# showlab/VideoSwap

Hardware: AMD Instinct MI355X
Metric: denoised frames/sec, 16-frame 512x512 clip @ 50 DDIM steps (end to end: inversion + CFG sampling) (higher is better)
Workload: dtype f16; 1 GPU; BASELINE.json configs[1]: 16-frame 512x512 clip, SD-1.5 UNet3D + AnimateDiff motion modules, 50-step DDIM inversion (B=1) + 50-step CFG-7.5 DDIM sampling (B=2), 1 clip per GPU per step; launch=eager, parallelism=clip-parallel x1

## Files before the change

include/vsx.h:

```cpp
#ifndef VSX_H_
#define VSX_H_

#include <stddef.h>
#include <stdint.h>

#ifdef __cplusplus
extern "C" {
#endif

#define VSX_ABI_VERSION 14

#define VSX_OK 0
#define VSX_E_BADSHAPE (-1)
#define VSX_E_UNSUPPORTED (-2)
#define VSX_E_LAUNCH (-3)
#define VSX_E_WORKSPACE (-4)

typedef void* vsx_stream_t;

int vsx_abi_version(void);
const char* vsx_last_error(void);
const char* vsx_source_digest(void);
int vsx_set_option(const char* name, int64_t value);

// ... 28 lines not shown
    double alpha;
    void* workspace;
    int64_t workspace_bytes;
    int64_t pad_lo, pad_hi;
    const void* rowscale;
    const void* colvec;
    void* rowstats;
    int64_t rowstats_parts;
} vsx_gemm_desc;

int vsx_gemm_f16(const vsx_gemm_desc* d, vsx_stream_t stream);
int64_t vsx_gemm_rowstats_parts(const vsx_gemm_desc* d);
int64_t vsx_gemm_workspace(const vsx_gemm_desc* d);

int64_t vsx_groupnorm_chunks(int64_t rows, int64_t nimg);
int vsx_groupnorm_stats(const void* x1, const void* x2, int64_t nimg, int64_t rows, int64_t C1,
                        int64_t C2, int64_t groups, float* partial, vsx_stream_t stream);
int vsx_groupnorm_apply(const void* x1, const void* x2, int64_t nimg, int64_t rows, int64_t C1,
                        int64_t C2, int64_t groups, const float* partial, int64_t nchunks,
                        int64_t count_rows, const void* gamma, const void* beta, float eps,
                        int64_t silu, float* stats, void* y, vsx_stream_t stream);

int vsx_row_stats(const void* x, int64_t M, int64_t C, float eps, float* stats, vsx_stream_t stream);
int vsx_row_stats_combine(const float* parts, int64_t M, int64_t nparts, int64_t C, float eps, float* stats,
                          vsx_stream_t stream);

int vsx_layernorm(const void* x, int64_t M, int64_t C, const void* gamma, const void* beta,
                  float eps, const void* pe, int64_t rows_per_frame, int64_t frames,
                  int64_t frame_offset, void* y, vsx_stream_t stream);

int vsx_attention_f16(const void* Q, const void* K, const void* VT, void* O, int64_t nb,
                      int64_t heads, int64_t nq, int64_t nk, int64_t d, int64_t ldq, int64_t ldk,
                      int64_t ldvt, int64_t ldo, int64_t q_bs, int64_t k_bs, int64_t vt_bs,
                      int64_t o_bs, int64_t kv_div, float scale, vsx_stream_t stream);

int vsx_attention_lse_f16(const void* Q, const void* K, const void* VT, void* O, float* lse, int64_t lse_ld, int64_t nb,
                          int64_t heads, int64_t nq, int64_t nk, int64_t d, int64_t ldq, int64_t ldk, int64_t ldvt,
                          int64_t ldo, int64_t q_bs, int64_t k_bs, int64_t vt_bs, int64_t o_bs, int64_t kv_div,
                          float scale, vsx_stream_t stream);
int64_t vsx_attention_bwd_supported(int64_t d);
int vsx_attention_bwd_f16(const void* Q, const void* K, const void* V, const void* O, const void* dO, const void* QT,
                          const void* KT, const void* dOT, const float* lse, float* delta, void* dQ, void* dK, void* dV,
                          int64_t nb, int64_t heads, int64_t nq, int64_t nk, int64_t d, int64_t ldtq, int64_t ldtk,
                          int64_t lds, int64_t kv_div, float scale, vsx_stream_t stream);

int vsx_softmax_rows(void* S, int64_t nrows, int64_t ncols, int64_t ld, vsx_stream_t stream);
int vsx_softmax_rows_causal(void* S, int64_t nrows, int64_t ncols, int64_t ld, int64_t rows_per_seq,
                            vsx_stream_t stream);

int vsx_temporal_attention_f16(const void* Q, const void* K, const void* V, void* O, int64_t B,
                               int64_t fq, int64_t fk, int64_t hw, int64_t heads, int64_t d,
                               int64_t ldq, int64_t ldkv, int64_t ldo, float scale,
                               vsx_stream_t stream);

int vsx_silu(const void* x, void* y, int64_t n, vsx_stream_t stream);
int vsx_quick_gelu(const void* x, void* y, int64_t n, vsx_stream_t stream);
int vsx_axpy(const void* a, const void* b, float s, void* y, int64_t n, vsx_stream_t stream);
int vsx_pack_latents(const void* x, void* y, int64_t B, int64_t Cin, int64_t F, int64_t HW,
                     int64_t Cpad, vsx_stream_t stream);
int vsx_unpack_latents(const void* x, void* y, int64_t B, int64_t Cout, int64_t F, int64_t HW,
                       int64_t Cs, vsx_stream_t stream);
int vsx_cfg_ddim_step(const void* x, const void* eps_u, const void* eps_c, float guidance,
                      float alpha_t, float alpha_next, void* out, int64_t n, vsx_stream_t stream);
int vsx_masked_blend(const void* x, const void* src, const void* mask, void* out, int64_t C,
                     int64_t n_sp, vsx_stream_t stream);

int vsx_adapter_scatter(const float* tracks, const int32_t* selected, const void* feat, void* out,
                        int64_t F, int64_t P, int64_t C, int64_t h, int64_t w, float rate,
                        float out_scale, vsx_stream_t stream);

int vsx_prof_enable(int64_t on, int64_t max_samples);
int vsx_prof_pause(int64_t paused);
int vsx_prof_collect(int64_t* n_launches, double* total_ms, double* total_flop);
int vsx_prof_collect_roofline(double peak_flops, double peak_bytes_per_s, int64_t* n_launches, double* total_ms,
                              double* total_flop, double* total_bytes, double* floor_ms, double* byte_bound_ms);

#define VSX_COMM_OP_SEND 1
#define VSX_COMM_OP_RECV 2
#define VSX_COMM_OP_ALLGATHER 3
#define VSX_COMM_OP_ALLREDUCE 4
#define VSX_COMM_OP_LOCAL_COPY 5
#define VSX_COMM_OP_GROUP_START 6
#define VSX_COMM_OP_GROUP_END 7
int vsx_comm_unique_id(void* id128);
int vsx_comm_init(int64_t rank, int64_t nranks, const void* id128);
int vsx_comm_init_recording(int64_t rank, int64_t nranks);
int64_t vsx_comm_recorded(int64_t* out, int64_t capacity);
int64_t vsx_comm_size(void);
int64_t vsx_comm_rank(void);
int vsx_comm_destroy(void);
int vsx_allgather_kv(const void* kv_local, void* kv_all, int64_t batch, int64_t elems_per_batch,
                     vsx_stream_t stream);
int vsx_allgather_f32(const float* local, float* all, int64_t count, vsx_stream_t stream);
int vsx_allreduce_gnstats(float* partial, int64_t count, vsx_stream_t stream);
int vsx_alltoall_f16(const void* send, void* recv, int64_t nouter, int64_t ninner, int64_t block_elems,
                     const int64_t* send_strides, const int64_t* recv_strides, vsx_stream_t stream);

int vsx_geglu_fwd(const void* y2, void* out, int64_t M, int64_t N, vsx_stream_t stream);
int vsx_geglu_bwd(const void* dout, const void* y2, void* dy2, int64_t M, int64_t N, vsx_stream_t stream);
int vsx_silu_bwd(const void* dy, const void* x, void* dx, int64_t n, vsx_stream_t stream);
int64_t vsx_groupnorm_bwd_workspace(int64_t nimg, int64_t rows, int64_t groups);
int vsx_groupnorm_bwd(const void* dy, const void* x1, const void* x2, int64_t nimg, int64_t rows, int64_t C1,
                      int64_t C2, int64_t groups, const void* gamma, const void* beta, float eps, int64_t silu,
                      void* ws, void* dx1, void* dx2, vsx_stream_t stream);
int vsx_layernorm_bwd(const void* dy, const void* x, const void* gamma, float eps, void* dx, int64_t M, int64_t C,
                      vsx_stream_t stream);
// ... 42 lines not shown
```

videoswap_amd/_lib.py:

```python
import ctypes
import os
from ctypes import POINTER, Structure, c_char_p, c_double, c_float, c_int, c_int32, c_int64, c_void_p

_HERE = os.path.dirname(os.path.abspath(__file__))
VARIANT = os.environ.get('VSX_LIB_VARIANT') or None
LIB_PATH = os.path.join(_HERE, 'lib', 'libvsx.so' if not VARIANT else f'libvsx_{VARIANT}.so')

VSX_ABI_VERSION = 14
VSX_E_UNSUPPORTED = -2


class VsxError(RuntimeError):
    pass


class GemmDesc(Structure):

    def __init__(self, *args, **kwargs):
        super().__init__(*args, **kwargs)
        if 'pad_lo' not in kwargs:
            self.pad_lo = -1
        if 'pad_hi' not in kwargs:
            self.pad_hi = -1

    _fields_ = [
        ('M', c_int64), ('N', c_int64), ('K', c_int64),
        ('batch0', c_int64), ('batch1', c_int64),
        ('A', c_void_p), ('A2', c_void_p),
        ('lda', c_int64), ('a_bs0', c_int64), ('a_bs1', c_int64),
        ('a_mode', c_int64), ('H', c_int64), ('W', c_int64), ('C1', c_int64), ('C2', c_int64),
        ('ks', c_int64), ('stride', c_int64), ('upsample', c_int64),
        ('B', c_void_p), ('ldb', c_int64), ('b_bs0', c_int64), ('b_bs1', c_int64),
        ('C', c_void_p), ('ldc', c_int64), ('c_bs0', c_int64), ('c_bs1', c_int64),
        ('c_mode', c_int64), ('c_rows_per_img', c_int64), ('c_img_stride', c_int64),
        ('bias', c_void_p), ('rowvec', c_void_p), ('rows_per_vec', c_int64),
        ('residual', c_void_p), ('ldr', c_int64), ('r_bs0', c_int64), ('r_bs1', c_int64),
        ('geglu', c_int64), ('alpha', c_double),
        ('workspace', c_void_p), ('workspace_bytes', c_int64),
        ('pad_lo', c_int64), ('pad_hi', c_int64),
        ('rowscale', c_void_p), ('colvec', c_void_p),
        ('rowstats', c_void_p), ('rowstats_parts', c_int64),
    ]


PROTOTYPES = {
    'vsx_abi_version': (c_int, []),
    'vsx_last_error': (c_char_p, []),
    'vsx_source_digest': (c_char_p, []),
    'vsx_set_option': (c_int, [c_char_p, c_int64]),
    'vsx_gemm_f16': (c_int, [POINTER(GemmDesc), c_void_p]),
    'vsx_gemm_workspace': (c_int64, [POINTER(GemmDesc)]),
    'vsx_gemm_rowstats_parts': (c_int64, [POINTER(GemmDesc)]),
    'vsx_groupnorm_chunks': (c_int64, [c_int64, c_int64]),
    'vsx_groupnorm_stats': (c_int, [c_void_p, c_void_p, c_int64, c_int64, c_int64, c_int64, c_int64, c_void_p,
                                    c_void_p]),
    'vsx_groupnorm_apply': (c_int, [c_void_p, c_void_p, c_int64, c_int64, c_int64, c_int64, c_int64, c_void_p,
                                    c_int64, c_int64, c_void_p, c_void_p, c_float, c_int64, c_void_p, c_void_p, c_void_p]),
    'vsx_row_stats': (c_int, [c_void_p, c_int64, c_int64, c_float, c_void_p, c_void_p]),
    'vsx_row_stats_combine': (c_int, [c_void_p, c_int64, c_int64, c_int64, c_float, c_void_p, c_void_p]),
    'vsx_layernorm': (c_int, [c_void_p, c_int64, c_int64, c_void_p, c_void_p, c_float, c_void_p, c_int64, c_int64,
                              c_int64, c_void_p, c_void_p]),
    'vsx_attention_f16': (c_int, [c_void_p, c_void_p, c_void_p, c_void_p] + [c_int64] * 14 + [c_float, c_void_p]),
    'vsx_attention_lse_f16': (c_int, [c_void_p, c_void_p, c_void_p, c_void_p, c_void_p] + [c_int64] * 15 + [c_float, c_void_p]),
    'vsx_attention_bwd_supported': (c_int64, [c_int64]),
    'vsx_attention_bwd_f16': (c_int, [c_void_p] * 13 + [c_int64] * 9 + [c_float, c_void_p]),
    'vsx_softmax_rows': (c_int, [c_void_p, c_int64, c_int64, c_int64, c_void_p]),
    'vsx_softmax_rows_causal': (c_int, [c_void_p, c_int64, c_int64, c_int64, c_int64, c_void_p]),
    'vsx_temporal_attention_f16': (c_int, [c_void_p, c_void_p, c_void_p, c_void_p] + [c_int64] * 9
                                   + [c_float, c_void_p]),
    'vsx_silu': (c_int, [c_void_p, c_void_p, c_int64, c_void_p]),
    'vsx_quick_gelu': (c_int, [c_void_p, c_void_p, c_int64, c_void_p]),
    'vsx_axpy': (c_int, [c_void_p, c_void_p, c_float, c_void_p, c_int64, c_void_p]),
    'vsx_pack_latents': (c_int, [c_void_p, c_void_p, c_int64, c_int64, c_int64, c_int64, c_int64, c_void_p]),
    'vsx_unpack_latents': (c_int, [c_void_p, c_void_p, c_int64, c_int64, c_int64, c_int64, c_int64, c_void_p]),
    'vsx_cfg_ddim_step': (c_int, [c_void_p, c_void_p, c_void_p, c_float, c_float, c_float, c_void_p, c_int64,
                                  c_void_p]),
    'vsx_masked_blend': (c_int, [c_void_p, c_void_p, c_void_p, c_void_p, c_int64, c_int64, c_void_p]),
    'vsx_adapter_scatter': (c_int, [c_void_p, c_void_p, c_void_p, c_void_p, c_int64, c_int64, c_int64, c_int64,
                                    c_int64, c_float, c_float, c_void_p]),
    'vsx_prof_enable': (c_int, [c_int64, c_int64]),
    'vsx_comm_unique_id': (c_int, [c_void_p]),
    'vsx_comm_init': (c_int, [c_int64, c_int64, c_void_p]),
    'vsx_comm_init_recording': (c_int, [c_int64, c_int64]),
    'vsx_comm_recorded': (c_int64, [POINTER(c_int64), c_int64]),
    'vsx_comm_size': (c_int64, []),
    'vsx_comm_rank': (c_int64, []),
    'vsx_comm_destroy': (c_int, []),
    'vsx_allgather_kv': (c_int, [c_void_p, c_void_p, c_int64, c_int64, c_void_p]),
    'vsx_allgather_f32': (c_int, [c_void_p, c_void_p, c_int64, c_void_p]),
    'vsx_allreduce_gnstats': (c_int, [c_void_p, c_int64, c_void_p]),
    'vsx_prof_pause': (c_int, [c_int64]),
    'vsx_prof_collect': (c_int, [POINTER(c_int64), POINTER(c_double), POINTER(c_double)]),
    'vsx_prof_collect_roofline': (c_int, [c_double, c_double, POINTER(c_int64), POINTER(c_double), POINTER(c_double),
                                          POINTER(c_double), POINTER(c_double), POINTER(c_double)]),
    'vsx_geglu_fwd': (c_int, [c_void_p, c_void_p, c_int64, c_int64, c_void_p]),
    'vsx_geglu_bwd': (c_int, [c_void_p, c_void_p, c_void_p, c_int64, c_int64, c_void_p]),
    'vsx_silu_bwd': (c_int, [c_void_p, c_void_p, c_void_p, c_int64, c_void_p]),
    'vsx_groupnorm_bwd_workspace': (c_int64, [c_int64, c_int64, c_int64]),
    'vsx_groupnorm_bwd': (c_int, [c_void_p, c_void_p, c_void_p, c_int64, c_int64, c_int64, c_int64, c_int64, c_void_p,
                                  c_void_p, c_float, c_int64, c_void_p, c_void_p, c_void_p, c_void_p]),
    'vsx_layernorm_bwd': (c_int, [c_void_p, c_void_p, c_void_p, c_float, c_void_p, c_int64, c_int64, c_void_p]),
    'vsx_softmax_bwd': (c_int, [c_void_p, c_void_p, c_int64, c_int64, c_int64, c_float, c_void_p]),
    'vsx_sum_pool2x2': (c_int, [c_void_p, c_void_p, c_int64, c_int64, c_int64, c_int64, c_void_p]),
    'vsx_adapter_gather': (c_int, [c_void_p, c_void_p, c_void_p, c_void_p, c_int64, c_int64, c_int64, c_int64, c_int64,
                                   c_float, c_float, c_void_p]),
    'vsx_alltoall_f16': (c_int, [c_void_p, c_void_p, c_int64, c_int64, c_int64, POINTER(c_int64), POINTER(c_int64),
                                 c_void_p]),
    'vsx_dift_sample_points': (c_int, [c_void_p] + [c_int64] * 7 + [c_void_p, c_int64, c_void_p, c_int64, c_void_p,
                                                                       c_void_p, c_void_p]),
    'vsx_dift_cosine_map_workspace': (c_int64, [c_int64] * 5),
    'vsx_dift_cosine_map': (c_int, [c_void_p] + [c_int64] * 7 + [c_void_p, c_int64, c_int64, c_void_p, c_int64,
                                                                    c_void_p, c_void_p, c_void_p, c_void_p]),
    'vsx_coord_mlp_f32': (c_int, [c_void_p] + [c_int64] * 10 + [c_void_p, c_int64, c_void_p, c_void_p]),
    'vsx_hash_grid_geometry': (c_int64, [c_int64] * 4 + [c_double] + [c_void_p] * 5),
    'vsx_hash_grid_f32': (c_int, [c_void_p, c_int64, c_int64, c_void_p] + [c_int64] * 5 + [c_double, c_void_p, c_void_p]),
    'vsx_hash_mlp_f32': (c_int, [c_void_p, c_int64, c_int64, c_void_p] + [c_int64] * 5 + [c_double] + [c_int64] * 5
                         + [c_void_p, c_int64, c_void_p, c_void_p]),
    'vsx_atlas_edit_f32': (c_int, [c_void_p, c_void_p, c_void_p, c_int64]
                           + ([c_void_p] + [c_int64] * 3 + [c_float] * 3 + [c_void_p, c_void_p, c_int64, c_int64]) * 2
                           + [c_void_p] * 5),
}

# ... 43 lines not shown
```

videoswap_amd/attention.py:

```python
import torch
from torch import nn

from . import ops
from .layers import Identity, Linear, StepInvariantCache


class Attention(nn.Module):
    def __init__(self, query_dim, cross_attention_dim=None, heads=8, dim_head=64, dropout=0.0, bias=False,
                 upcast_attention=False, upcast_softmax=False, out_bias=True, scale_qk=True,
                 only_cross_attention=False, rescale_output_factor=1.0, residual_connection=False, processor=None,
                 **unsupported):
        super().__init__()
        if upcast_attention or upcast_softmax or dropout != 0.0 or unsupported:
            raise NotImplementedError(f'Attention: unsupported options {unsupported or "upcast/dropout"}')
        inner_dim = dim_head * heads
        cross_attention_dim = cross_attention_dim if cross_attention_dim is not None else query_dim
        self.upcast_attention = False
        self.upcast_softmax = False
        self.rescale_output_factor = rescale_output_factor
        self.residual_connection = residual_connection
        self.scale_qk = scale_qk
        self.scale = dim_head ** -0.5 if scale_qk else 1.0
        self.heads = heads
        self.sliceable_head_dim = heads
# ... 177 lines not shown
        return self.pe[0]


class VanillaAttentionProcessor(nn.Module):
    vsx_native = True

    @property
    def vsx_graph_safe(self):
        return self.kv_gather is None

    def __init__(self, attention_mode=None, cross_frame_attention_mode=None, temporal_position_encoding=False,
                 temporal_position_encoding_max_len=24, attention_op=None, *args, **kwargs):
        super().__init__()
        self.attention_op = attention_op
        self.attention_mode = attention_mode
        self.is_cross_attention = kwargs.get('cross_attention_dim') is not None
        if attention_mode != 'Temporal' or self.is_cross_attention:
            raise NotImplementedError('only Temporal_Self attention blocks exist in the VideoSwap configs')
        self.pos_encoder = PositionalEncoding(kwargs['query_dim'], dropout=0.0,
                                              max_len=temporal_position_encoding_max_len) \
            if temporal_position_encoding else None
        self.kv_gather = None

    @property
    def frame_offset(self):
        g = self.kv_gather
        return g.frame_offset if g is not None and g.kv_active else 0

    def pe_table(self):
        return None if self.pos_encoder is None else self.pos_encoder.table()

    def __call__(self, attn, hidden_states, encoder_hidden_states=None, attention_mask=None, temb=None,
                 video_length=None, residual=None, pe_applied=False):
        bf, hw, c = hidden_states.shape
        frames = video_length
        b = bf // frames
        x = hidden_states
        if self.pos_encoder is not None and not pe_applied:
            pe = self.pe_table()[self.frame_offset:self.frame_offset + frames].to(x.dtype)
            x = (x.view(b, frames, hw, c) + pe[None, :, None, :]).view(bf, hw, c)
        nobias = attn.to_q.bias is None and attn.to_k.bias is None and attn.to_v.bias is None
        fk = frames
        if self.kv_gather is not None and self.kv_gather.kv_active:
            if nobias:
                kv = ops.linear(x, attn.fused_weight(('to_k', 'to_v'))).view(-1, 2 * c)
            else:
                kv = torch.cat([attn.to_k(x).view(-1, c), attn.to_v(x).view(-1, c)], dim=1)
            handle = self.kv_gather.kv_gather_start(kv, b, frames, hw)
            q = attn.to_q(x).view(-1, c)
            kv_all, fk = self.kv_gather.kv_gather_finish(handle)
            k, v = kv_all[:, :c], kv_all[:, c:]
        elif nobias:
            qkv = ops.linear(x, attn.fused_weight(('to_q', 'to_k', 'to_v'))).view(-1, 3 * c)
            q, k, v = qkv[:, :c], qkv[:, c:2 * c], qkv[:, 2 * c:]
        else:
            q, k, v = attn.to_q(x).view(-1, c), attn.to_k(x).view(-1, c), attn.to_v(x).view(-1, c)
        o = ops.temporal_attention(q, k, v, b, frames, fk, hw, attn.heads, attn.scale).view(bf, hw, c)
        return attn.to_out[0](o, residual=residual, row_stats=True)
```

videoswap_amd/build.py:

```python
import hashlib
import os
import re
import shutil
import subprocess
import sys
import tempfile
from concurrent.futures import ThreadPoolExecutor

HERE = os.path.dirname(os.path.abspath(__file__))
ROOT = os.path.dirname(HERE)
CSRC = os.path.join(HERE, 'csrc')
LIBDIR = os.path.join(HERE, 'lib')
OBJDIR = os.path.join(LIBDIR, 'obj')
LIB = os.path.join(LIBDIR, 'libvsx.so')
VARIANTS = {}
VARIANT_EXTRA = {}
SOURCES = ['api.cpp', 'comm.cpp', 'options.cpp', 'prof.cpp', 'gemm.hip', 'gemm_pp.hip', 'norm.hip', 'attention.hip', 'attention_bwd.hip', 'elementwise.hip',
           'train.hip', 'dift.hip', 'atlas.hip', 'atlas_edit.hip']
HIPCC = os.environ.get('HIPCC', '/opt/rocm/bin/hipcc')
FLAGS = ['--offload-arch=gfx950', '-O3', '-std=c++17', '-fPIC', '-x', 'hip',
         '-I', os.path.join(ROOT, 'include'), '-I', CSRC, '-Wall', '-Wno-unused-function', '-Wno-division-by-zero',
         '-mllvm', '-amdgpu-mfma-vgpr-form']


def lib_path(variant=None):
    return LIB if not variant else os.path.join(LIBDIR, f'libvsx_{variant}.so')


def _digest(variant=None):
    h = hashlib.sha256()
    swap = VARIANTS[variant] if variant else {}
    names = [n for n in sorted(os.listdir(CSRC)) if n.endswith(('.hip', '.cpp', '.h'))]
    for name in names + ['../../include/vsx.h']:
        with open(os.path.join(CSRC, swap.get(name, name)), 'rb') as f:
            h.update(name.encode() + b'\0' + f.read())
    h.update(' '.join(f.replace(ROOT, '<root>') for f in FLAGS).encode())
    if variant:
        for name in VARIANT_EXTRA.get(variant, []):
            with open(os.path.join(CSRC, name), 'rb') as f:
                h.update(name.encode() + b'\0' + f.read())
        h.update(b'\0variant ' + variant.encode())
    return h.hexdigest()


def source_digest(variant=None):
    return _digest(variant)


_MARKER = b'@vsx-source-digest:'


def built_digest(variant=None):
    path = lib_path(variant)
    if not os.path.exists(path):
        return None
    with open(path, 'rb') as f:
        blob = f.read()
    i = blob.find(_MARKER)
    if i < 0:
        return None
    j = blob.find(b'\0', i)
    return blob[i + len(_MARKER):j].decode(errors='replace')


def _compile(src, digest, variant=None):
    objdir = OBJDIR if not variant else os.path.join(LIBDIR, f'obj_{variant}')
    os.makedirs(objdir, exist_ok=True)
    obj = os.path.join(objdir, src.replace('/', '_') + '.o')
    extra = [f'-DVSX_SOURCE_DIGEST="{digest}"'] if src == 'api.cpp' else []
    path = os.path.join(CSRC, (VARIANTS[variant] if variant else {}).get(src, src))
    cmd = [HIPCC] + FLAGS + extra + ['-c', path, '-o', obj]
    r = subprocess.run(cmd, capture_output=True, text=True)
    if r.returncode != 0:
        raise RuntimeError(f'hipcc failed for {src}:\n{r.stdout}\n{r.stderr}')
    if r.stderr.strip():
        sys.stderr.write(r.stderr)
    return obj


LLVM_BIN = os.environ.get('VSX_LLVM_BIN', '/opt/rocm/lib/llvm/bin')
NO_SCRATCH = ('gemm_pp_kernel', 'gemm_ws320_kernel', 'flash_attn_kernel', 'gemm_kernelILi256E', 'coord_mlp_kernel')


def parse_kernel_notes(text):
    keys = ('vgpr_count', 'agpr_count', 'sgpr_count', 'vgpr_spill_count', 'sgpr_spill_count',
            'private_segment_fixed_size', 'group_segment_fixed_size')
    out, cur = {}, None
    for line in text.splitlines():
        m = re.match(r'^\s+(-\s+)?\.(\w+):\s*(\S.*)?$', line)
        if not m:
            continue
        if m.group(1) and re.match(r'^  - ', line):
            cur = {}
        if cur is None:
            continue
        key, val = m.group(2), (m.group(3) or '').strip()
        if key == 'name' and re.match(r'^    \.name:', line):
            out[val] = cur
        elif key in keys and re.match(r'^  (- |  )\.', line):
            cur[key] = int(val)
    return out


def kernel_resources(lib=None):
    lib = lib or LIB
    objdump, readelf = os.path.join(LLVM_BIN, 'llvm-objdump'), os.path.join(LLVM_BIN, 'llvm-readelf')
    tmp = tempfile.mkdtemp(prefix='vsx_co_')
    try:
        copy = os.path.join(tmp, 'lib.so')
        shutil.copy(lib, copy)
        r = subprocess.run([objdump, '--offloading', copy], capture_output=True, text=True, cwd=tmp)
        if r.returncode != 0:
            raise RuntimeError(f'llvm-objdump --offloading failed:\n{r.stderr}')
        res = {}
        for name in sorted(os.listdir(tmp)):
            if 'gfx950' not in name:
                continue
            r = subprocess.run([readelf, '--notes', os.path.join(tmp, name)], capture_output=True, text=True)
            if r.returncode != 0:
                raise RuntimeError(f'llvm-readelf --notes failed on {name}:\n{r.stderr}')
            res.update(parse_kernel_notes(r.stdout))
        return res
    finally:
        shutil.rmtree(tmp, ignore_errors=True)


def demangle(names):
    filt = shutil.which('c++filt') or shutil.which('llvm-cxxfilt')
    out = []
    if filt and names:
        r = subprocess.run([filt], input='\n'.join(names), capture_output=True, text=True)
        out = r.stdout.splitlines() if r.returncode == 0 else []
    return dict(zip(names, out if len(out) == len(names) else names))

# ... 126 lines not shown
```

videoswap_amd/csrc/options.cpp:

```cpp
#include "options.h"

#include <stdlib.h>
#include <string.h>

#include "common.h"

namespace vsxg {
namespace {
struct Option { const char* name; const char* env; long value; bool init; };
Option g_options[] = {{"gemm_pp", "VSX_GEMM_PP", 1, false}, {"pp_sched", "VSX_PP_SCHED", 0, false},
                      {"tile_tune", "VSX_TUNE_TILE", 0, false}, {"xcd_walk", "VSX_XCD_WALK", 1, false},
                      {"attn_qb", "VSX_ATTN_QB", 0, false}, {"temporal_out", "VSX_TEMPORAL_OUT", 0, false},
                      {"attn_o16", "VSX_ATTN_O16", 0, false}, {"gn_fuse", "VSX_GN_FUSE", 0, false},
                      {"gemm_ws", "VSX_GEMM_WS", 1, false}, {"ws_waves", "VSX_WS_WAVES", 10, false}};
Option* find_option(const char* name) {
    for (auto& o : g_options)
        if (strcmp(o.name, name) == 0) {
            if (!o.init) {
                const char* e = getenv(o.env);
                if (e) o.value = atol(e);
                o.init = true;
            }
            return &o;
        }
    return nullptr;
}
}
long gemm_option(const char* name) {
    Option* o = find_option(name);
    return o ? o->value : 0;
}
}

extern "C" int vsx_set_option(const char* name, int64_t value) {
    auto* o = name ? vsxg::find_option(name) : nullptr;
    if (!o) return vsx_fail(VSX_E_BADSHAPE, "vsx_set_option: unknown option '%s'", name ? name : "(null)");
    o->value = (long)value;
    return VSX_OK;
}
```

videoswap_amd/ops.py:

```python
import ctypes
import os

import torch

from . import _lib
from ._lib import GemmDesc, check

_F16 = torch.float16


_raw_stream = getattr(torch._C, '_cuda_getCurrentRawStream', None)


def _stream():
    if _raw_stream is not None:
        return ctypes.c_void_p(_raw_stream(torch.cuda.current_device()))
    return ctypes.c_void_p(torch.cuda.current_stream().cuda_stream)


def _p(t):
    return None if t is None else ctypes.c_void_p(t.data_ptr())


def _chk(t, name, dtype=_F16):
# ... 452 lines not shown
    _chk_view(t, name)
    if t.dim() != 3 or t.stride(2) != 1 or t.stride(1) % 8 or t.stride(0) % 8 or (t.data_ptr() % 16):
        raise _lib.VsxError(f'{name}: need unit inner stride, 16-byte aligned base, strides multiple of 8 (got {t.stride()})')
    return t.stride(1), t.stride(0)


def _chk_view(t, name):
    if not t.is_cuda or t.dtype != _F16:
        raise _lib.VsxError(f'{name}: expected an fp16 GPU tensor')


def attention(q, k, vt, heads, scale, kv_div=1, nk=None):
    _chk(vt, 'vt')
    ldq, q_bs = _rows_view(q, 'q')
    ldk, k_bs = _rows_view(k, 'k')
    nb, nq, C = q.shape
    nk = k.shape[1] if nk is None else nk
    dh = C // heads
    out = torch.empty(nb, nq, C, dtype=_F16, device=q.device)
    if FlopCounter.enabled:
        FlopCounter.attention += 4.0 * nb * heads * nq * nk * dh
    check(_lib.load().vsx_attention_f16(_p(q), _p(k), _p(vt), _p(out), nb, heads, nq, nk, dh, ldq, ldk, vt.shape[2], C,
                                        q_bs, k_bs, C * vt.shape[2], nq * C, kv_div, float(scale),
                                        _stream()), 'vsx_attention_f16')
    return out


def temporal_attention(q, k, v, B, fq, fk, hw, heads, scale):
    for t, n in ((q, 'q'), (k, 'k'), (v, 'v')):
        _chk_view(t, n)
        if t.dim() != 2 or t.stride(1) != 1 or t.stride(0) % 8 or t.data_ptr() % 16:
            raise _lib.VsxError(f'{n}: need a [rows, C] tensor with unit inner stride and aligned rows')
    if k.stride(0) != v.stride(0):
        raise _lib.VsxError('temporal_attention: k and v must share their row stride')
    C = q.shape[-1]
    out = torch.empty(q.shape[0], C, dtype=_F16, device=q.device)
    if FlopCounter.enabled:
        FlopCounter.attention += 4.0 * B * hw * fq * fk * C
    fn = _lib.load().vsx_temporal_attention_f16
    if fq <= 32 or fk > 128:
        check(fn(_p(q), _p(k), _p(v), _p(out), B, fq, fk, hw, heads, C // heads, q.stride(0), k.stride(0), C,
                 float(scale), _stream()), 'vsx_temporal_attention_f16')
        return out
    for b in range(B):
        kb, vb = k[b * fk * hw:(b + 1) * fk * hw], v[b * fk * hw:(b + 1) * fk * hw]
        for f0 in range(0, fq, 32):
            n = min(32, fq - f0)
            r0 = (b * fq + f0) * hw
            check(fn(_p(q[r0:r0 + n * hw]), _p(kb), _p(vb), _p(out[r0:r0 + n * hw]), 1, n, fk, hw, heads, C // heads,
                     q.stride(0), k.stride(0), C, float(scale), _stream()), 'vsx_temporal_attention_f16')
    return out


def group_norm(x, gamma, beta, groups, eps, nimg, silu=False, x2=None, partial_hook=None, count_rows=None):
    _chk(x, 'x'); _chk(x2, 'x2'); _chk(gamma, 'gamma'); _chk(beta, 'beta')
    C1 = x.shape[-1]
    C2 = x2.shape[-1] if x2 is not None else 0
    rows = x.numel() // C1 // nimg
    lib = _lib.load()
    nchunks = lib.vsx_groupnorm_chunks(rows, nimg)
    partial = torch.empty(nimg, nchunks, groups, 2, dtype=torch.float32, device=x.device)
    s = _stream()
    check(lib.vsx_groupnorm_stats(_p(x), _p(x2), nimg, rows, C1, C2, groups, _p(partial), s), 'vsx_groupnorm_stats')
    if partial_hook is not None:
        partial = partial_hook(partial)
        nchunks = partial.shape[1]
    y = torch.empty(*x.shape[:-1], C1 + C2, dtype=_F16, device=x.device)
    stats = torch.empty(nimg, groups, 2, dtype=torch.float32, device=x.device)
    check(lib.vsx_groupnorm_apply(_p(x), _p(x2), nimg, rows, C1, C2, groups, _p(partial), nchunks,
                                  rows if count_rows is None else count_rows, _p(gamma), _p(beta), float(eps),
                                  1 if silu else 0, _p(stats), _p(y), s), 'vsx_groupnorm_apply')
    return y


def layer_norm(x, gamma, beta, eps=1e-5, pe=None, rows_per_frame=0, frames=0, frame_offset=0):
    if isinstance(x, DeferredLN):
        raise _lib.VsxError('layer_norm of a deferred LayerNorm: materialize() it first')
    _chk(x, 'x'); _chk(gamma, 'gamma'); _chk(beta, 'beta'); _chk(pe, 'pe')
    C = x.shape[-1]
    if pe is not None:
        if pe.dim() != 2 or pe.shape[1] != C or frames <= 0 or rows_per_frame <= 0 or frame_offset < 0 \
                or pe.shape[0] < frame_offset + frames:
            raise _lib.VsxError(f'layer_norm: positional-encoding table {tuple(pe.shape)} does not cover frames '
                                f'[{frame_offset}, {frame_offset + frames}) x {C} channels')
    y = torch.empty_like(x)
    check(_lib.load().vsx_layernorm(_p(x), x.numel() // C, C, _p(gamma), _p(beta), float(eps), _p(pe), rows_per_frame,
                                    frames, frame_offset, _p(y), _stream()), 'vsx_layernorm')
    return y


def silu(x):
    _chk(x, 'x')
    y = torch.empty_like(x)
    check(_lib.load().vsx_silu(_p(x), _p(y), x.numel(), _stream()), 'vsx_silu')
    return y


def quick_gelu(x):
    _chk(x, 'x')
    y = torch.empty_like(x)
    check(_lib.load().vsx_quick_gelu(_p(x), _p(y), x.numel(), _stream()), 'vsx_quick_gelu')
    return y


def axpy(a, b, s=1.0):
    _chk(a, 'a'); _chk(b, 'b')
# ... 427 lines not shown
```

Measured before the change: 4.274 frames/s.

## Fuse temporal attention with output projection, bias, residual and row stats for C=320

Adds a persistent HIP kernel for the 320-channel, 8-head, 16-frame temporal attention blocks. Each block loads packed q|k|v rows into LDS, runs attention with MFMA, then multiplies by the to_out weight held in registers. The same kernel adds bias and residual and writes per-row statistics for the following layernorm. This removes the separate attention-output round trip through HBM and the extra GEMM and epilogue launches, at the cost of a highly specialized kernel with tight LDS and register budgets that only applies to large M (>=65536) by default.

```diff
diff --git a/include/vsx.h b/include/vsx.h
--- a/include/vsx.h
+++ b/include/vsx.h
@@ -104,6 +104,10 @@
                                int64_t fq, int64_t fk, int64_t hw, int64_t heads, int64_t d,
                                int64_t ldq, int64_t ldkv, int64_t ldo, float scale,
                                vsx_stream_t stream);
+int vsx_temporal_attention_out_f16(const void* Q, const void* K, const void* V, int64_t ldq, int64_t ldkv, const void* W,
+                                   const void* bias, const void* residual, int64_t ldr, void* out, int64_t ldo,
+                                   float* rowstats, int64_t rowstats_parts, int64_t b, int64_t frames, int64_t hw,
+                                   int64_t heads, int64_t d, float scale, vsx_stream_t stream);
 
 int vsx_silu(const void* x, void* y, int64_t n, vsx_stream_t stream);
 int vsx_quick_gelu(const void* x, void* y, int64_t n, vsx_stream_t stream);
diff --git a/videoswap_amd/_lib.py b/videoswap_amd/_lib.py
--- a/videoswap_amd/_lib.py
+++ b/videoswap_amd/_lib.py
@@ -68,6 +68,8 @@
     'vsx_softmax_rows_causal': (c_int, [c_void_p, c_int64, c_int64, c_int64, c_int64, c_void_p]),
     'vsx_temporal_attention_f16': (c_int, [c_void_p, c_void_p, c_void_p, c_void_p] + [c_int64] * 9
                                    + [c_float, c_void_p]),
+    'vsx_temporal_attention_out_f16': (c_int, [c_void_p, c_void_p, c_void_p, c_int64, c_int64, c_void_p, c_void_p, c_void_p,
+                                               c_int64, c_void_p, c_int64, c_void_p] + [c_int64] * 6 + [c_float, c_void_p]),
     'vsx_silu': (c_int, [c_void_p, c_void_p, c_int64, c_void_p]),
     'vsx_quick_gelu': (c_int, [c_void_p, c_void_p, c_int64, c_void_p]),
     'vsx_axpy': (c_int, [c_void_p, c_void_p, c_float, c_void_p, c_int64, c_void_p]),
diff --git a/videoswap_amd/attention.py b/videoswap_amd/attention.py
--- a/videoswap_amd/attention.py
+++ b/videoswap_amd/attention.py
@@ -253,6 +253,14 @@
             k, v = kv_all[:, :c], kv_all[:, c:]
         elif nobias:
             qkv = ops.linear(x, attn.fused_weight(('to_q', 'to_k', 'to_v'))).view(-1, 3 * c)
+            to_out = attn.to_out[0]
+            if (c == 320 and attn.heads == 8 and frames == 16 and residual is not None and ops.ROW_STATS_FROM_PRODUCER and qkv.is_cuda
+                    and type(to_out) is Linear and not (torch.is_grad_enabled() and (
+                        qkv.requires_grad or residual.requires_grad or to_out.weight.requires_grad))):
+                out = ops.temporal_attention_out(qkv, to_out.weight, to_out.bias, residual, b, frames, hw, attn.heads,
+                                                 attn.scale, shape=(bf, hw, c))
+                if out is not None:
+                    return out
             q, k, v = qkv[:, :c], qkv[:, c:2 * c], qkv[:, 2 * c:]
         else:
             q, k, v = attn.to_q(x).view(-1, c), attn.to_k(x).view(-1, c), attn.to_v(x).view(-1, c)
diff --git a/videoswap_amd/build.py b/videoswap_amd/build.py
--- a/videoswap_amd/build.py
+++ b/videoswap_amd/build.py
@@ -15,7 +15,7 @@
 LIB = os.path.join(LIBDIR, 'libvsx.so')
 VARIANTS = {}
 VARIANT_EXTRA = {}
-SOURCES = ['api.cpp', 'comm.cpp', 'options.cpp', 'prof.cpp', 'gemm.hip', 'gemm_pp.hip', 'norm.hip', 'attention.hip', 'attention_bwd.hip', 'elementwise.hip',
+SOURCES = ['api.cpp', 'comm.cpp', 'options.cpp', 'prof.cpp', 'gemm.hip', 'gemm_pp.hip', 'norm.hip', 'attention.hip', 'temporal_out.hip', 'attention_bwd.hip', 'elementwise.hip',
            'train.hip', 'dift.hip', 'atlas.hip', 'atlas_edit.hip']
 HIPCC = os.environ.get('HIPCC', '/opt/rocm/bin/hipcc')
 FLAGS = ['--offload-arch=gfx950', '-O3', '-std=c++17', '-fPIC', '-x', 'hip',
@@ -79,7 +79,7 @@
 
 
 LLVM_BIN = os.environ.get('VSX_LLVM_BIN', '/opt/rocm/lib/llvm/bin')
-NO_SCRATCH = ('gemm_pp_kernel', 'gemm_ws320_kernel', 'flash_attn_kernel', 'gemm_kernelILi256E', 'coord_mlp_kernel')
+NO_SCRATCH = ('gemm_pp_kernel', 'gemm_ws320_kernel', 'flash_attn_kernel', 'gemm_kernelILi256E', 'coord_mlp_kernel', 'temporal_out320_kernel')
 
 
 def parse_kernel_notes(text):
diff --git a/videoswap_amd/csrc/options.cpp b/videoswap_amd/csrc/options.cpp
--- a/videoswap_amd/csrc/options.cpp
+++ b/videoswap_amd/csrc/options.cpp
@@ -12,7 +12,8 @@
                       {"tile_tune", "VSX_TUNE_TILE", 0, false}, {"xcd_walk", "VSX_XCD_WALK", 1, false},
                       {"attn_qb", "VSX_ATTN_QB", 0, false}, {"temporal_out", "VSX_TEMPORAL_OUT", 0, false},
                       {"attn_o16", "VSX_ATTN_O16", 0, false}, {"gn_fuse", "VSX_GN_FUSE", 0, false},
-                      {"gemm_ws", "VSX_GEMM_WS", 1, false}, {"ws_waves", "VSX_WS_WAVES", 10, false}};
+                      {"gemm_ws", "VSX_GEMM_WS", 1, false}, {"ws_waves", "VSX_WS_WAVES", 10, false},
+                      {"temporal_fuse", "VSX_TEMPORAL_FUSE", 1, false}};
 Option* find_option(const char* name) {
     for (auto& o : g_options)
         if (strcmp(o.name, name) == 0) {
diff --git a/videoswap_amd/csrc/temporal_out.hip b/videoswap_amd/csrc/temporal_out.hip
--- /dev/null
+++ b/videoswap_amd/csrc/temporal_out.hip
@@ -0,0 +1,379 @@
+#include "gemm_common.h"
+
+namespace vsxg {
+namespace {
+
+struct TempOutParams {
+    const half_t* QKV;
+    const half_t* W;
+    const half_t* bias;
+    const half_t* residual;
+    half_t* out;
+    float* rowstats;
+    long ldr, ldo;
+    int parts;
+    int hw, bph, nblocks;
+    unsigned qkv_bytes;
+    float sl2;
+};
+
+constexpr int TO_NW = 10;
+constexpr int TO_F = 16, TO_D = 40, TO_C = 320;
+constexpr int TO_ROWB = 3 * TO_C * 2;
+constexpr int TO_FRB = 2 * TO_ROWB;
+constexpr int TO_SLOT = TO_F * TO_FRB;
+constexpr int TO_XP = TO_SLOT / 1024 / TO_NW;
+constexpr int TO_OT = 32 * 640;
+constexpr int TO_VT = 2 * 32 * 40 * 2;
+constexpr int TO_STG = 32 * 36 * 4;
+constexpr int TO_EXTRA = 2 * TO_SLOT;
+constexpr int TO_CST = TO_EXTRA + 2 * TO_STG;
+constexpr int TO_LDS = TO_CST + TO_NW * 128;
+constexpr int TO_WREG = 3 * 32 * 128;
+static_assert(TO_XP * TO_NW * 1024 == TO_SLOT, "the pieces of a block divide evenly among the waves");
+static_assert(TO_OT + 8 * TO_VT <= TO_SLOT && TO_STG <= TO_VT, "o tile and V^T / staging areas fit the slot being computed");
+static_assert(TO_NW * TO_WREG <= 2 * TO_SLOT && TO_LDS <= 160 * 1024, "LDS budget");
+
+__device__ __forceinline__ int to_fresh_lane(const int lane_hint) {
+    int l = lane_hint;
+    asm volatile("v_mbcnt_lo_u32_b32 %0, -1, 0\n\tv_mbcnt_hi_u32_b32 %0, -1, %0" : "=v"(l));
+    return l;
+}
+
+__device__ __forceinline__ int to_chunk(const int f, const int w) { return f * 3840 + ((w ^ f) << 4); }
+
+__device__ __forceinline__ int to_vt_col(const int key, const int chgroup) { return key ^ ((chgroup & 3) << 3); }
+
+__global__ __launch_bounds__(TO_NW * 64) void temporal_out320_kernel(const TempOutParams p) {
+    constexpr int RL = 2;
+    constexpr int OOB_OFF = (int)0x80000000;
+    constexpr int VSTR = 40;
+    extern __shared__ __attribute__((aligned(16))) unsigned char smem[];
+    const int tid = threadIdx.x;
+    const int lane = tid & 63;
+    const int wave = __builtin_amdgcn_readfirstlane(tid >> 6);
+    const int l31 = lane & 31, hi = lane >> 5;
+    const int lrow = lane >> 3, pslot = lane & 7;
+    const int chain = blockIdx.x, nchains = gridDim.x;
+    const int hw = p.hw, bph = p.bph;
+    int nmine = 0;
+    if (chain < p.nblocks) nmine = (p.nblocks - 1 - chain) / nchains + 1;
+    if (nmine == 0) return;
+
+    h8 wf[20];
+    {
+        const __amdgpu_buffer_rsrc_t rsrcW = __builtin_amdgcn_make_buffer_rsrc(const_cast<half_t*>(p.W), 0, TO_C * TO_C * 2, 0x00020000);
+        const int vw_e = lrow * (TO_C * 2) + (pslot ^ (lrow >> 1)) * 16;
+        const int vw_o = lrow * (TO_C * 2) + (pslot ^ (4 | (lrow >> 1))) * 16;
+        unsigned char* wreg = smem + wave * TO_WREG;
+        const int fw = l31 * 128 + ((hi ^ ((l31 >> 1) & 7)) * 16);
+        auto w_round = [&](const int sl0, const int nsl) {
+#pragma unroll
+            for (int sl = 0; sl < 3; ++sl)
+                if (sl < nsl)
+#pragma unroll
+                    for (int pc = 0; pc < 4; ++pc)
+                        __builtin_amdgcn_raw_ptr_buffer_load_lds(rsrcW, (lptr_t)(wreg + sl * 4096 + pc * 1024), 16, (pc & 1) ? vw_o : vw_e,
+                                                                 (32 * wave + 8 * pc) * (TO_C * 2) + (sl0 + sl) * 128, 0, 0);
+            wait_vmcnt<0>();
+            __builtin_amdgcn_sched_barrier(0);
+        };
+        w_round(0, 3);
+#pragma unroll
+        for (int t = 0; t < 12; ++t) wf[t] = *reinterpret_cast<const h8*>(wreg + (t >> 2) * 4096 + (fw ^ ((t & 3) * 32)));
+        asm volatile("s_waitcnt lgkmcnt(0)" ::: "memory");
+        __builtin_amdgcn_sched_barrier(0);
+        w_round(3, 2);
+#pragma unroll
+        for (int t = 12; t < 20; ++t) wf[t] = *reinterpret_cast<const h8*>(wreg + ((t >> 2) - 3) * 4096 + (fw ^ ((t & 3) * 32)));
+        asm volatile("s_waitcnt lgkmcnt(0)" ::: "memory");
+    }
+    const bool has_bias = p.bias != nullptr;
+    float* cst = reinterpret_cast<float*>(smem + TO_CST + wave * 128);
+    if (has_bias && lane < 8) {
+        const h4 cb = *reinterpret_cast<const h4*>(p.bias + 32 * wave + 4 * lane);
+        f4v bf;
+#pragma unroll
+        for (int e = 0; e < 4; ++e) bf[e] = (float)cb[e];
+        *reinterpret_cast<f4v*>(cst + 4 * lane) = bf;
+    }
+    __builtin_amdgcn_sched_barrier(0);
+    __builtin_amdgcn_s_barrier();
+    __builtin_amdgcn_sched_barrier(0);
+
+    const __amdgpu_buffer_rsrc_t rsrcX = __builtin_amdgcn_make_buffer_rsrc(const_cast<half_t*>(p.QKV), 0, (int)p.qkv_bytes, 0x00020000);
+    const unsigned frame_b = (unsigned)hw * (unsigned)TO_ROWB;
+    auto block_coords = [&](const int i, unsigned& row0, bool& two) {
+        const int blk = chain + i * nchains;
+        const int b = blk / bph, jj = blk - b * bph;
+        row0 = (unsigned)(b * TO_F) * (unsigned)hw + 2u * (unsigned)jj;
+        two = 2 * jj + 1 < hw;
+    };
+    auto issue_x = [&](const int i, const int lane) {
+        const bool on = i < nmine;
+        unsigned row0 = 0;
+        bool two = false;
+        block_coords(on ? i : 0, row0, two);
+        const unsigned base = row0 * (unsigned)TO_ROWB;
+        const int slot = (i & 1) * TO_SLOT;
+#pragma unroll
+        for (int k = 0; k < TO_XP; ++k) {
+            const int c = (wave * TO_XP + k) * 64 + lane;
+            const int f = c / 240, w = (c - f * 240) ^ f;
+            const bool take = on && (two || w < 120);
+            __builtin_amdgcn_raw_ptr_buffer_load_lds(rsrcX, (lptr_t)(smem + slot + (wave * TO_XP + k) * 1024), 16,
+                                                     take ? (int)(base + (unsigned)f * frame_b + (unsigned)w * 16u) : OOB_OFF, 0, 0, 0);
+        }
+    };
+    issue_x(0, lane);
+    wait_vmcnt<0>();
+
+    const int asite = min(wave >> 2, 1), head0 = (wave & 3) * 2;
+    unsigned char* priv = smem + (wave < 8 ? TO_OT + wave * TO_VT : TO_EXTRA + (wave - 8) * TO_STG);
+    const int lane_entry = lane;
+
+    int prev_stores = 0;
+    for (int j = 0; j < nmine; ++j) {
+        const int lane = to_fresh_lane(lane_entry);
+        const int l31 = lane & 31, hi = lane >> 5;
+        const int fa = l31 * 128 + ((hi ^ ((l31 >> 1) & 7)) * 16);
+        const int col8 = (lane & 3) * 8, r0 = lane >> 2;
+        const int ncol = 32 * wave + col8;
+        if (j > 0) {
+            if (prev_stores == 4) wait_vmcnt<4>();
+            else wait_vmcnt<2>();
+        }
+        __builtin_amdgcn_sched_barrier(0);
+        __builtin_amdgcn_s_barrier();
+        __builtin_amdgcn_sched_barrier(0);
+        unsigned row0 = 0;
+        bool two = false;
+        block_coords(j, row0, two);
+        h8 pre[RL];
+#pragma unroll
+        for (int ps = 0; ps < RL; ++ps) {
+            const size_t m = (size_t)row0 + (size_t)r0 * (unsigned)hw + (two ? ps : 0);
+            pre[ps] = *reinterpret_cast<const h8*>(p.residual + m * (size_t)p.ldr + ncol);
+        }
+        VSX_VMEM_NOTE(RL);
+        asm volatile("" ::: "memory");
+        __builtin_amdgcn_sched_barrier(0);
+        issue_x(j + 1, lane);
+        unsigned char* slot = smem + (j & 1) * TO_SLOT;
+        float* stg = reinterpret_cast<float*>(wave < 8 ? slot + (priv - smem) : priv);
+
+        const unsigned char* xs = slot;
+        const int wsite = asite * (TO_ROWB / 16);
+        h8 raw[3];
+        h8 ka[3], qb[3];
+        const int krow = (l31 & ~12) | ((l31 & 4) << 1) | ((l31 & 8) >> 1);
+        const int qg = l31 >> 4, qf_ = l31 & 15;
+        {
+#pragma unroll
+            for (int i = 0; i < 3; ++i) {
+                const int u = min(lane + 64 * i, 159);
+                const int key = u / 5, ch = u - key * 5;
+                const int g = key >> 4, f = key & 15;
+                raw[i] = *reinterpret_cast<const h8*>(xs + to_chunk(f, wsite + 80 + (head0 + g) * 5 + ch));
+            }
+            const int kg = krow >> 4, kf_ = krow & 15;
+            const int kw = wsite + 40 + (head0 + kg) * 5 + hi, qw = wsite + (head0 + qg) * 5 + hi;
+#pragma unroll
+            for (int t = 0; t < 3; ++t) {
+                const bool in = t * 16 + hi * 8 < TO_D;
+                const h8 kv = *reinterpret_cast<const h8*>(xs + to_chunk(kf_, kw + 2 * t)), qv = *reinterpret_cast<const h8*>(xs + to_chunk(qf_, qw + 2 * t));
+                ka[t] = in ? kv : h8{};
+                qb[t] = in ? qv : h8{};
+            }
+        }
+        asm volatile("s_waitcnt lgkmcnt(0)" ::: "memory");
+        __builtin_amdgcn_sched_barrier(0);
+        __builtin_amdgcn_s_barrier();
+        __builtin_amdgcn_sched_barrier(0);
+
+        if (wave < 8) {
+            half_t* sVT = reinterpret_cast<half_t*>(stg);
+#pragma unroll
+            for (int i = 0; i < 3; ++i) {
+                const int u = lane + 64 * i;
+                if (u < 160) {
+                    const int key = u / 5, ch = u - key * 5;
+                    const h8 v = raw[i];
+#pragma unroll
+                    for (int e = 0; e < 8; ++e) sVT[(ch * 8 + e) * VSTR + to_vt_col(key, ch)] = v[e];
+                }
+            }
+            const f16v zero = {0.f, 0.f, 0.f, 0.f, 0.f, 0.f, 0.f, 0.f, 0.f, 0.f, 0.f, 0.f, 0.f, 0.f, 0.f, 0.f};
+            f16v sc = zero;
+#pragma unroll
+            for (int t = 0; t < 3; ++t) sc = __builtin_amdgcn_mfma_f32_32x32x16_f16(ka[t], qb[t], t == 0 ? zero : sc, 0, 0, 0);
+            const int lo = qg * TO_F, up = lo + TO_F;
+            const float sl2 = p.sl2;
+            float mx = -INFINITY;
+#pragma unroll
+            for (int r = 0; r < 16; ++r) {
+                const int key = (r & 3) + 4 * ((r >> 2) & 1) + 8 * hi + 16 * (r >> 3);
+                const bool v = key >= lo && key < up;
+                sc[r] = v ? sc[r] * sl2 : -INFINITY;
+                mx = fmaxf(mx, sc[r]);
+            }
+            mx = fmaxf(mx, __shfl_xor(mx, 32, 64));
+            if (mx == -INFINITY) mx = 0.f;
+            float sum = 0.f;
+#pragma unroll
+            for (int r = 0; r < 16; ++r) {
+                sc[r] = __builtin_amdgcn_exp2f(sc[r] - mx);
+                sum += sc[r];
+            }
+            sum += __shfl_xor(sum, 32, 64);
+            const float inv = sum > 0.f ? 1.0f / sum : 0.f;
+            h8 pf[2];
+#pragma unroll
+            for (int s2 = 0; s2 < 2; ++s2)
+#pragma unroll
+                for (int jj = 0; jj < 8; ++jj) pf[s2][jj] = (half_t)sc[8 * s2 + jj];
+            __builtin_amdgcn_sched_barrier(0);
+            const int orow = asite * 16 + qf_;
+            unsigned char* ot = slot + orow * 128;
+            const int osw = (orow >> 1) & 7;
+#pragma unroll
+            for (int t = 0; t < 2; ++t) {
+                f16v o = zero;
+#pragma unroll
+                for (int s2 = 0; s2 < 2; ++s2) {
+                    const h8 vf = *reinterpret_cast<const h8*>(sVT + (t * 32 + l31) * VSTR + to_vt_col(16 * s2 + 8 * hi, (t * 32 + l31) >> 3));
+                    o = __builtin_amdgcn_mfma_f32_32x32x16_f16(vf, pf[s2], o, 0, 0, 0);
+                }
+#pragma unroll
+                for (int g4 = 0; g4 < 4; ++g4) {
+                    const int c = t * 32 + 8 * g4 + 4 * hi;
+                    if (c < TO_D) {
+                        h4 pk;
+#pragma unroll
+                        for (int e = 0; e < 4; ++e) pk[e] = (half_t)(o[4 * g4 + e] * inv);
+                        const int col = (head0 + qg) * TO_D + c;
+                        *reinterpret_cast<h4*>(ot + (col >> 6) * 4096 + ((((col & 63) >> 3) ^ osw) * 16) + (col & 7) * 2) = pk;
+                    }
+                }
+            }
+        }
+        asm volatile("s_waitcnt lgkmcnt(0)" ::: "memory");
+        __builtin_amdgcn_sched_barrier(0);
+        __builtin_amdgcn_s_barrier();
+        __builtin_amdgcn_sched_barrier(0);
+
+        f16v acc;
+        {
+            const f16v zero = {};
+            const h8 xf = *reinterpret_cast<const h8*>(slot + fa);
+            acc = __builtin_amdgcn_mfma_f32_32x32x16_f16(wf[0], xf, zero, 0, 0, 0);
+        }
+#pragma unroll
+        for (int t = 1; t < 20; ++t) {
+            const h8 xf = *reinterpret_cast<const h8*>(slot + (t >> 2) * 4096 + (fa ^ ((t & 3) * 32)));
+            acc = __builtin_amdgcn_mfma_f32_32x32x16_f16(wf[t], xf, acc, 0, 0, 0);
+        }
+#pragma unroll
+        for (int g = 0; g < 4; ++g) {
+            f4v v;
+#pragma unroll
+            for (int e = 0; e < 4; ++e) v[e] = acc[4 * g + e] * 1.0f;
+            *reinterpret_cast<f4v*>(stg + l31 * 36 + 8 * g + 4 * hi) = v;
+        }
+        __builtin_amdgcn_sched_barrier(0);
+        float bv[8];
+        if (has_bias) {
+            const f4v b0 = *reinterpret_cast<const f4v*>(cst + col8), b1 = *reinterpret_cast<const f4v*>(cst + col8 + 4);
+#pragma unroll
+            for (int e = 0; e < 4; ++e) { bv[e] = b0[e]; bv[e + 4] = b1[e]; }
+        }
+#pragma unroll
+        for (int ps = 0; ps < 2; ++ps) {
+            const int row = ps * 16 + r0;
+            const f4v a = *reinterpret_cast<const f4v*>(stg + row * 36 + col8);
+            const f4v b = *reinterpret_cast<const f4v*>(stg + row * 36 + col8 + 4);
+            float ov[8] = {a[0], a[1], a[2], a[3], b[0], b[1], b[2], b[3]};
+            if (has_bias) {
+#pragma unroll
+                for (int e = 0; e < 8; ++e) ov[e] += bv[e];
+            }
+            const h8 add = pre[ps];
+#pragma unroll
+            for (int e = 0; e < 8; ++e) ov[e] += (float)add[e];
+            h8 pk;
+#pragma unroll
+            for (int e = 0; e < 8; ++e) pk[e] = (half_t)ov[e];
+            const h2 one2 = {(half_t)1.f, (half_t)1.f};
+            float s1 = 0.f, s2 = 0.f;
+#pragma unroll
+            for (int e = 0; e < 8; e += 2) {
+                const h2 v = {pk[e], pk[e + 1]};
+                s1 = __builtin_amdgcn_fdot2(v, one2, s1, false);
+                s2 = __builtin_amdgcn_fdot2(v, v, s2, false);
+            }
+#pragma unroll
+            for (int d = 2; d > 0; d >>= 1) {
+                s1 += __shfl_xor(s1, d, 64);
+                s2 += __shfl_xor(s2, d, 64);
+            }
+            if (ps == 0 || two) {
+                const size_t m = (size_t)row0 + (size_t)r0 * (unsigned)hw + ps;
+                *reinterpret_cast<h8*>(p.out + m * (size_t)p.ldo + ncol) = pk;
+                typedef float f2v __attribute__((ext_vector_type(2)));
+                float* sp = p.rowstats + (m * (unsigned)p.parts + (unsigned)wave) * 2;
+                if (col8 == 0) *reinterpret_cast<f2v*>(sp) = f2v{s1, s2};
+            }
+        }
+        prev_stores = two ? 4 : 2;
+        VSX_VMEM_NOTE(prev_stores);
+        __builtin_amdgcn_sched_barrier(0);
+    }
+}
+
+}
+}
+
+extern "C" int vsx_temporal_attention_out_f16(const void* Q, const void* K, const void* V, int64_t ldq, int64_t ldkv, const void* W,
+                                              const void* bias, const void* residual, int64_t ldr, void* out, int64_t ldo,
+                                              float* rowstats, int64_t rowstats_parts, int64_t b, int64_t frames, int64_t hw,
+                                              int64_t heads, int64_t d, float scale, vsx_stream_t stream) {
+    using namespace vsxg;
+    VSX_REQUIRE(Q && K && V && W && out, VSX_E_BADSHAPE, "temporal_attention_out: null tensor");
+    VSX_REQUIRE(b >= 0 && hw >= 0 && frames > 0 && heads > 0 && d > 0, VSX_E_BADSHAPE, "temporal_attention_out: bad sizes");
+    const long fuse = gemm_option("temporal_fuse");
+    const long M = (long)(b * frames * hw);
+    const half_t* q = (const half_t*)Q;
+    const bool shape = heads == 8 && d == TO_D && frames == TO_F && ldq == 3 * TO_C && ldkv == 3 * TO_C &&
+                       (const half_t*)K == q + TO_C && (const half_t*)V == q + 2 * TO_C && residual != nullptr && rowstats != nullptr &&
+                       rowstats_parts == TO_NW && ldr >= TO_C && ldo >= TO_C && ldr % 8 == 0 && ldo % 8 == 0 && vsx_aligned16(Q) &&
+                       vsx_aligned16(W) && vsx_aligned16(bias) && vsx_aligned16(residual) && vsx_aligned16(out) &&
+                       ((uintptr_t)rowstats & 7) == 0 && (unsigned long)M * TO_ROWB < (1ul << 31) &&
+                       (unsigned long)M * (unsigned long)(ldr > ldo ? ldr : ldo) * 2ul < (1ul << 40);
+    if (!shape || fuse == 0 || (fuse == 1 && M < 65536))
+        return vsx_fail(VSX_E_UNSUPPORTED, "temporal_attention_out: not the fused shape (C = 320, 8 heads of 40, 16 frames, q|k|v in one "
+                                           "[M, 960] buffer, residual and 10 statistics parts) or temporal_fuse = %ld", fuse);
+    if (M == 0) return VSX_OK;
+    static bool attr_set = false;
+    if (!attr_set) {
+        hipError_t e = hipFuncSetAttribute(reinterpret_cast<const void*>(&temporal_out320_kernel), hipFuncAttributeMaxDynamicSharedMemorySize, TO_LDS);
+        if (e != hipSuccess) return vsx_fail(VSX_E_LAUNCH, "temporal_attention_out: hipFuncSetAttribute: %s", hipGetErrorString(e));
+        attr_set = true;
+    }
+    static int n_cu = 0;
+    if (n_cu == 0) {
+        int dev = 0;
+        hipDeviceProp_t prop;
+        if (hipGetDevice(&dev) != hipSuccess || hipGetDeviceProperties(&prop, dev) != hipSuccess)
+            return vsx_fail(VSX_E_LAUNCH, "temporal_attention_out: cannot query the device");
+        n_cu = prop.multiProcessorCount > 0 ? prop.multiProcessorCount : 256;
+    }
+    TempOutParams p;
+    p.QKV = q; p.W = (const half_t*)W; p.bias = (const half_t*)bias; p.residual = (const half_t*)residual;
+    p.out = (half_t*)out; p.rowstats = rowstats; p.ldr = ldr; p.ldo = ldo; p.parts = (int)rowstats_parts;
+    p.hw = (int)hw; p.bph = (int)((hw + 1) / 2); p.nblocks = (int)(b * p.bph);
+    p.qkv_bytes = (unsigned)((unsigned long)M * TO_ROWB);
+    p.sl2 = scale * 1.44269504088896340736f;
+    const int grid = p.nblocks < n_cu ? p.nblocks : n_cu;
+    hipLaunchKernelGGL(temporal_out320_kernel, dim3((unsigned)grid), dim3(TO_NW * 64), TO_LDS, (hipStream_t)stream, p);
+    return vsx_check_launch("vsx_temporal_attention_out_f16");
+}
diff --git a/videoswap_amd/ops.py b/videoswap_amd/ops.py
--- a/videoswap_amd/ops.py
+++ b/videoswap_amd/ops.py
@@ -528,6 +528,33 @@
     return out
 
 
+TEMPORAL_OUT_PARTS = 10
+
+
+def temporal_attention_out(qkv, weight, bias, residual, B, frames, hw, heads, scale, shape=None):
+    _chk(qkv, 'qkv'); _chk(weight, 'weight'); _chk(bias, 'bias'); _chk(residual, 'residual')
+    if qkv.dim() != 2 or qkv.shape[1] % 3 or weight.dim() != 2:
+        return None
+    M, C = qkv.shape[0], qkv.shape[1] // 3
+    if weight.shape != (C, C) or residual.numel() != M * C or M != B * frames * hw or C % heads:
+        return None
+    out = torch.empty(*(shape or (M, C)), dtype=_F16, device=qkv.device)
+    parts = torch.empty(M, TEMPORAL_OUT_PARTS, 2, dtype=torch.float32, device=qkv.device)
+    base, esz = qkv.data_ptr(), qkv.element_size()
+    rc = _lib.load().vsx_temporal_attention_out_f16(
+        ctypes.c_void_p(base), ctypes.c_void_p(base + C * esz), ctypes.c_void_p(base + 2 * C * esz), 3 * C, 3 * C, _p(weight),
+        _p(bias), _p(residual), C, _p(out), C, _p(parts), TEMPORAL_OUT_PARTS, B, frames, hw, heads, C // heads, float(scale),
+        _stream())
+    if rc == _lib.VSX_E_UNSUPPORTED:
+        return None
+    check(rc, 'vsx_temporal_attention_out_f16')
+    if FlopCounter.enabled:
+        FlopCounter.attention += 4.0 * B * hw * frames * frames * C
+        FlopCounter.gemm += 2.0 * M * C * C
+    out._vsx_rowparts = parts
+    return out
+
+
 def group_norm(x, gamma, beta, groups, eps, nimg, silu=False, x2=None, partial_hook=None, count_rows=None):
     _chk(x, 'x'); _chk(x2, 'x2'); _chk(gamma, 'gamma'); _chk(beta, 'beta')
     C1 = x.shape[-1]
```

New measurement: 4.293 frames/s, median of 6. About the same (+0.4%).
